# ihsanhadi57/Face-Detection-With-YOLOv11-SAHI-and-Real-ESRGAN

Hardware: AMD Instinct MI355X
Metric: end-to-end 4K frames/sec (SAHI+YOLOv11s+ESRGAN×4) (higher is better)
Workload: dtype f32x3(detect)+f16(sr)

## Files before the change

face-detection-with-yolov11-sahi-and-real-esrgan_amd/build.py:

```python
from __future__ import annotations

import os
import shutil
import subprocess
import sys
from concurrent.futures import ThreadPoolExecutor

HERE = os.path.dirname(os.path.abspath(__file__))
CSRC = os.path.join(HERE, "csrc")
OUT = os.path.join(HERE, "libffp.so")
SOURCES = ["common.cpp", "weights.cpp", "engine.cpp", "conv_route.cpp", "conv_mfma.hip", "conv_rows.hip", "conv_rows16.hip", "conv_rows16pc.hip", "conv_trunk.hip", "conv_pw.hip", "conv_k3d.hip", "conv_dwpw.hip", "ops_misc.hip", "det_post.hip", "merge.hip", "eval.hip", "coco_eval.hip", "iqa.hip", "jpeg.hip", "jpeg_huff.hip", "jpeg_dec.cpp", "png.hip", "png_dec.cpp", "png_dec.hip", "overlay.hip",
           "sr_ops.hip", "resize.hip", "yolo11.cpp", "rrdb.cpp", "onnx_graph.cpp", "scrfd_ops.hip", "scrfd.cpp", "rtdetr_ops.hip", "rtdetr.cpp", "sliced.cpp", "api.cpp",
           "api_eval.cpp", "api_codec.cpp", "api_ops.cpp"]
FLAGS = ["-O3", "-std=c++17", "--offload-arch=gfx950", "-fPIC", "-Wall", "-Wno-unused-function", "-Wno-unused-result",
         "-ffp-contract=off"]


def _hipcc() -> str:
    for c in (os.environ.get("HIPCC"), shutil.which("hipcc"), "/opt/rocm/bin/hipcc"):
        if c and os.path.exists(c):
            return c
    raise RuntimeError("hipcc not found (ROCm toolchain required to build libffp.so)")


# ... 72 lines not shown
        base = _obj_base(s_)
        if s_ in srcs:
            obj = os.path.join(bdir, f"{base}.{name}.o")
            cmd = [_hipcc(), *FLAGS, *defs, "-c", os.path.join(CSRC, s_), "-o", obj]
            r = subprocess.run(cmd, capture_output=True, text=True)
            if r.returncode != 0:
                raise RuntimeError(f"hipcc failed on {s_} ({name}):\n{r.stdout}\n{r.stderr}")
            objs.append(obj)
        else:
            objs.append(os.path.join(bdir, base + ".o"))
    out = os.path.join(bdir, f"libffp_{name}.so")
    r = subprocess.run([_hipcc(), "--offload-arch=gfx950", "-shared", "-fPIC", "-o", out, *objs], capture_output=True, text=True)
    if r.returncode != 0:
        raise RuntimeError(f"link failed:\n{r.stdout}\n{r.stderr}")
    if verbose:
        print(f"built {out}")
    return out


ASAN_SOURCES = ["common.cpp", "weights.cpp", "jpeg_dec.cpp", "png_dec.cpp", "onnx_graph.cpp", "asan_host_check.cpp"]
ASAN_OUT = os.path.join(CSRC, "build", "asan_host_check")


def build_asan(verbose: bool = True) -> str:
    clang = os.path.join(os.path.dirname(os.path.realpath(_hipcc())), "..", "lib", "llvm", "bin", "clang++")
    if not os.path.exists(clang):
        clang = "/opt/rocm/lib/llvm/bin/clang++"
    os.makedirs(os.path.dirname(ASAN_OUT), exist_ok=True)
    srcs = [os.path.join(CSRC, s) for s in ASAN_SOURCES]
    if os.path.exists(ASAN_OUT) and os.path.getmtime(ASAN_OUT) > max(max(os.path.getmtime(s) for s in srcs), _newest_header()):
        return ASAN_OUT
    cmd = [clang, "-std=c++17", "-O1", "-g", "-fsanitize=address,undefined", "-fno-sanitize-recover=undefined", "-fno-omit-frame-pointer",
           "-D__HIP_PLATFORM_AMD__", "-I/opt/rocm/include", *srcs, "-o", ASAN_OUT, "-L/opt/rocm/lib", "-lamdhip64", "-Wl,-rpath,/opt/rocm/lib"]
    r = subprocess.run(cmd, capture_output=True, text=True)
    if r.returncode != 0:
        raise RuntimeError(f"sanitizer build failed:\n{r.stdout}\n{r.stderr}")
    if verbose:
        print(f"built {ASAN_OUT}")
    return ASAN_OUT


def _build_host_check(out: str, driver: str, headers: list, verbose: bool, sanitize: tuple = ("-fsanitize=address,undefined", "-fno-sanitize-recover=undefined")) -> str:
    clang = os.path.join(os.path.dirname(os.path.realpath(_hipcc())), "..", "lib", "llvm", "bin", "clang++")
    if not os.path.exists(clang):
        clang = "/opt/rocm/lib/llvm/bin/clang++"
    out = os.path.join(CSRC, "build", out)
    os.makedirs(os.path.dirname(out), exist_ok=True)
    srcs = [os.path.join(CSRC, f) for f in [driver, *headers]]
    if os.path.exists(out) and os.path.getmtime(out) > max(os.path.getmtime(s) for s in srcs):
        return out
    cmd = [clang, "-std=c++17", "-O1", "-g", "-Wall", *sanitize, "-fno-omit-frame-pointer", srcs[0], "-o", out]
    r = subprocess.run(cmd, capture_output=True, text=True)
    if r.returncode != 0:
        raise RuntimeError(f"sanitizer build failed:\n{r.stdout}\n{r.stderr}")
    if verbose:
        print(f"built {out}")
    return out


def build_arena_check(verbose: bool = True) -> str:
    return _build_host_check("arena_host_check", "arena_host_check.cpp", ["arena.hpp"], verbose)


def build_dw_bound_check(verbose: bool = True) -> str:
    return _build_host_check("dw_bound_host_check", "dw_bound_host_check.cpp", ["dw_bound.hpp"], verbose)


def build_plan_cache_check(verbose: bool = True) -> str:
    return _build_host_check("plan_cache_host_check", "plan_cache_host_check.cpp", ["plan_cache.hpp"], verbose)


def build_switches_check(verbose: bool = True) -> str:
    return _build_host_check("switches_host_check", "switches_host_check.cpp", ["switches.hpp"], verbose)


def build_jpeg_batch_plan_check(verbose: bool = True) -> str:
    return _build_host_check("jpeg_batch_plan_host_check", "jpeg_batch_plan_host_check.cpp", ["jpeg_batch_plan.hpp"], verbose)


def build_sr_tiles_check(verbose: bool = True) -> str:
    return _build_host_check("sr_tiles_host_check", "sr_tiles_host_check.cpp", ["sr_tiles.hpp"], verbose)


def build_ws_pool_check(verbose: bool = True) -> tuple:
    args = ("ws_pool_host_check.cpp", ["ws_pool.hpp"], verbose)
    return (_build_host_check("ws_pool_host_check_asan", *args, sanitize=("-pthread", "-fsanitize=address,undefined", "-fno-sanitize-recover=undefined")),
            _build_host_check("ws_pool_host_check_tsan", *args, sanitize=("-pthread", "-fsanitize=thread")))


if __name__ == "__main__":
    if "--asan" in sys.argv:
        build_asan()
    elif "--arena-check" in sys.argv:
        build_arena_check()
    elif "--dw-bound-check" in sys.argv:
        build_dw_bound_check()
    elif "--plan-cache-check" in sys.argv:
        build_plan_cache_check()
    elif "--switches-check" in sys.argv:
        build_switches_check()
    elif "--jpeg-batch-plan-check" in sys.argv:
        build_jpeg_batch_plan_check()
    elif "--sr-tiles-check" in sys.argv:
        build_sr_tiles_check()
    elif "--ws-pool-check" in sys.argv:
        build_ws_pool_check()
    elif "--variant" in sys.argv:
        build_variant(sys.argv[sys.argv.index("--variant") + 1])
    else:
        build(force="--force" in sys.argv)
```

face-detection-with-yolov11-sahi-and-real-esrgan_amd/csrc/conv_route.cpp:

```cpp
#include "conv_route.hpp"

#include <algorithm>

#include "api_util.hpp"
#include "conv_args.hpp"
#include "engine.hpp"
#include "trunk.hpp"

namespace ffp {

namespace {

using F = ConvFamily;
constexpr ConvShapeInfo kShapes[SHAPE_COUNT] = {
    {SHAPE_WIDE, F::GENERIC, "generic", "wide"},         {SHAPE_WIDE_H, F::GENERIC, "generic", "wideH"},
    {SHAPE_NARROW2, F::GENERIC, "generic", "narrow2"},   {SHAPE_NARROW2_H, F::GENERIC, "generic", "narrow2H"},
    {SHAPE_NARROW1, F::GENERIC, "generic", "narrow1"},   {SHAPE_NARROW1_H, F::GENERIC, "generic", "narrow1H"},
    {SHAPE_ROWS, F::ROWS, "rows", "rows"},               {SHAPE_ROWS_3STAGE, F::ROWS, "rows", "rows"},
    {SHAPE_ROWS_2TILE, F::ROWS, "rows", "rows"},         {SHAPE_ROWS16, F::ROWS16, "rows16", "rows16"},
    {SHAPE_PW_1X4, F::PW, "pw", "pw1x4"},                {SHAPE_PW_2X2, F::PW, "pw", "pw2x2"},
    {SHAPE_PW_2X1, F::PW, "pw", "pw2x1"},                {SHAPE_PW_1X4W, F::PW, "pw", "pw1x4w"},
    {SHAPE_PW_2X2W, F::PW, "pw", "pw2x2w"},              {SHAPE_PW_2X1W, F::PW, "pw", "pw2x1w"},
    {SHAPE_PW_1X4S, F::PW, "pw", "pw1x4s"},              {SHAPE_K3D_128, F::K3D, "k3d", "d128"},
    {SHAPE_K3D_64, F::K3D, "k3d", "d64"},                {SHAPE_K3D_32, F::K3D, "k3d", "d32"},
    {SHAPE_K3D_128X256, F::K3D, "k3d", "d128x256"},      {SHAPE_K3D_64X256, F::K3D, "k3d", "d64x256"},
    {SHAPE_PW_2X2S, F::PW, "pw", "pw2x2s"},              {SHAPE_ROWS16_RES, F::ROWS16, "rows16", "rows16"},
    {SHAPE_ROWS16PC, F::ROWS16PC, "rows16pc", "rows16pc"}, {SHAPE_TRUNK, F::TRUNK, "trunk", "trunk"},
};
constexpr ConvShapeInfo kDwPw{SHAPE_DWPW, F::DWPW, "dwpw", "dw3"};
constexpr bool table_in_order() {
  for (int i = 0; i < SHAPE_COUNT; ++i) if (kShapes[i].shape != i) return false;
  return true;
}
static_assert(table_in_order(), "conv shape table: row i holds shape i");
static_assert(SHAPE_COUNT <= 32 && SHAPE_DWPW >= 32, "forceable shapes fit a 32-bit candidate mask; route-only numbers lie above them");

bool family_runs(ConvFamily family, int shape, const ConvOp& op, const ConvArgs& a) {
  switch (family) {
    case F::GENERIC: return true;
    case F::ROWS: return conv_rows_eligible(op, a, shape);
    case F::ROWS16:
    case F::ROWS16PC: return conv_rows16_eligible(op, a, shape);
    case F::PW: return conv_pw_mask(op, a) & shape_bit(shape);
    case F::K3D: return conv_k3d_mask(op, a) & shape_bit(shape);
    case F::TRUNK: return conv_trunk_layer_ok(op);
    case F::DWPW: return conv_dwpw_eligible(op);
    case F::DIRECT: break;
  }
  return false;
}

}

const ConvShapeInfo* conv_shape_info(int shape) {
  if (shape < 0 || shape >= SHAPE_COUNT) return nullptr;
  return &kShapes[shape];
}

const ConvShapeInfo* conv_route_info(int shape) { return shape == SHAPE_DWPW ? &kDwPw : conv_shape_info(shape); }

ConvArgs conv_route_args(const ConvOp& op) { return op.dw || conv_direct_eligible(op) ? ConvArgs{} : make_conv_args(op); }

ConvRoute conv_route(const ConvOp& op, const ConvArgs& a) {
  if (op.dw) {
    FFP_CHECK((op.force_shape < 0 || op.force_shape == SHAPE_DWPW) && conv_dwpw_eligible(op), FFP_ERR_ARG, "conv %s: the depthwise-fused kernel cannot run this op", op.pc->name.c_str());
    return {F::DWPW, SHAPE_DWPW};
  }
  if (conv_direct_eligible(op)) {
    FFP_CHECK(!op.gate, FFP_ERR_ARG, "conv %s: the image-input kernel cannot honour a gate", op.pc->name.c_str());
    return {F::DIRECT, SHAPE_AUTO};
  }
  if (op.force_shape >= 0) {
    const ConvShapeInfo* s = conv_shape_info(op.force_shape);
    FFP_CHECK(s, FFP_ERR_ARG, "conv %s: %d is not a shape number", op.pc->name.c_str(), op.force_shape);
    FFP_CHECK(family_runs(s->family, s->shape, op, a), FFP_ERR_ARG, "conv %s: %s shape %d cannot run this op", op.pc->name.c_str(), s->family_name, s->shape);
    return {s->family, s->shape};
  }
  if (sw().rows16 && conv_rows16_eligible(op, a, SHAPE_ROWS16)) {
    if (sw().rows16_pc && a.dbg == 0) return {F::ROWS16PC, SHAPE_ROWS16PC};
    if (sw().rows16_res && conv_rows16_eligible(op, a, SHAPE_ROWS16_RES)) return {F::ROWS16, SHAPE_ROWS16_RES};
    return {F::ROWS16, SHAPE_ROWS16};
  }
  if (conv_rows_eligible(op, a, SHAPE_ROWS)) return {F::ROWS, SHAPE_ROWS};
  return {F::GENERIC, conv_generic_choose(op, a)};
}

unsigned conv_candidates(const ConvOp& op, const ConvArgs& a) {
  return conv_generic_mask(op, a) | (sw().pw ? conv_pw_mask(op, a) : 0u) | (sw().k3d ? conv_k3d_mask(op, a) : 0u);
}

void launch_conv(const ConvOp& op, hipStream_t st) {
  ConvArgs a = conv_route_args(op);
  const ConvRoute r = conv_route(op, a);
  switch (r.family) {
    case F::DIRECT: launch_conv_direct(op, st); return;
    case F::GENERIC: launch_conv_generic(a, r.shape, op, st); break;
    case F::ROWS: launch_conv_rows(a, r.shape, op.out.lvl, st); break;
    case F::ROWS16: launch_conv_rows16(a, r.shape, *op.pc, op.out.lvl, st); break;
    case F::ROWS16PC: launch_conv_rows16pc(a, *op.pc, op.out.lvl, st); break;
    case F::PW: launch_conv_pw(a, r.shape, st); break;
    case F::K3D: launch_conv_k3d(a, r.shape, op.stride, op.out.lvl, st); break;
    case F::DWPW: launch_conv_dwpw(op, st); break;
    case F::TRUNK: {
      TrunkPlan tp(std::vector<ConvOp>{op});
      tp.launch(st, op.dbg);
      FFP_HIP(hipStreamSynchronize(st));
      return;
    }
  }
  FFP_HIP(hipGetLastError());
}

std::string conv_variant(const ConvOp& op) {
  const PackedConv& pc = *op.pc;
  const ConvRoute r = conv_route(op, conv_route_args(op));
  if (r.family == F::DIRECT) return std::string(pc.dt == F32 ? "f32" : "f16") + "_k3_direct";
  char buf[64];
  snprintf(buf, sizeof(buf), "%s_k%ds%d_%s", pc.dt == F16 ? "f16" : pc.split ? "f32x3" : "f32", pc.k, op.stride, conv_route_info(r.shape)->suffix);
  return buf;
}

int conv_tune(const ConvOp& op, hipStream_t st) {
  const PackedConv& pc = *op.pc;
  const ConvArgs a = conv_route_args(op);
  const ConvRoute r = conv_route(op, a);
  if (op.force_shape >= 0 || r.family != F::GENERIC) return -1;
  const unsigned mask = conv_candidates(op, a);
  if (__builtin_popcount(mask) < 2) return -1;
  const int heur = r.shape;
  ScopedEvent e0, e1;
  auto time_shape = [&](int shape, int iters) {
    ConvOp o = op;
    o.force_shape = shape;
    o.gate = nullptr;
    FFP_HIP(hipEventRecord(e0, st));
    for (int i = 0; i < iters; ++i) launch_conv(o, st);
    FFP_HIP(hipEventRecord(e1, st));
    FFP_HIP(hipEventSynchronize(e1));
    float ms = 0.f;
    FFP_HIP(hipEventElapsedTime(&ms, e0, e1));
    return ms * 1e3f / iters;
  };
  float best_t = 0.f, heur_t = 0.f;
  int best = -1;
  for (int shape = 0; shape < SHAPE_COUNT; ++shape) {
    if (!(mask & shape_bit(shape))) continue;
    const float t1 = time_shape(shape, 2);
    const int iters = std::min(24, std::max(3, (int)(300.f / std::max(t1, 1.f))));
    const float t = time_shape(shape, iters);
    if (shape == heur) heur_t = t;
    if (best < 0 || t < best_t) { best = shape; best_t = t; }
    if (sw().tune_log) {
      ConvOp o = op;
      o.force_shape = shape;
      fprintf(stderr, "[tune] %-28s %4d->%4d k%d s%d px %9lld  shape %2d %-22s %9.1f us%s\n", pc.name.c_str(), pc.cin_real, pc.cout, pc.k, op.stride,
              (long long)op.out.lvl->actual_px(), shape, conv_variant(o).c_str(), t, shape == heur ? "  (heuristic)" : "");
    }
  }
  if (heur_t > 0.f && best_t > 0.97f * heur_t) return heur;
  return best;
}

}
// ... 1 lines not shown
```

face-detection-with-yolov11-sahi-and-real-esrgan_amd/csrc/conv_route.hpp:

```cpp
#pragma once
#include "ops.hpp"

namespace ffp {

struct ConvArgs;

enum ConvShape : int {
  SHAPE_AUTO = -1,
  SHAPE_WIDE = 0, SHAPE_WIDE_H, SHAPE_NARROW2, SHAPE_NARROW2_H, SHAPE_NARROW1, SHAPE_NARROW1_H,
  SHAPE_ROWS = 6, SHAPE_ROWS_3STAGE, SHAPE_ROWS_2TILE,
  SHAPE_ROWS16 = 9,
  SHAPE_PW_1X4 = 10, SHAPE_PW_2X2, SHAPE_PW_2X1, SHAPE_PW_1X4W, SHAPE_PW_2X2W, SHAPE_PW_2X1W,
  SHAPE_PW_1X4S = 16,
  SHAPE_K3D_128 = 17, SHAPE_K3D_64, SHAPE_K3D_32, SHAPE_K3D_128X256, SHAPE_K3D_64X256,
  SHAPE_PW_2X2S = 22,
  SHAPE_ROWS16_RES = 23,
  SHAPE_ROWS16PC = 24,
  SHAPE_TRUNK = 25,
  SHAPE_COUNT,
  SHAPE_DWPW = 64
};
constexpr unsigned shape_bit(int shape) { return 1u << shape; }

enum class ConvFamily { DIRECT, GENERIC, ROWS, ROWS16, ROWS16PC, PW, K3D, TRUNK, DWPW };

struct ConvShapeInfo { int shape; ConvFamily family; const char* family_name; const char* suffix; };
const ConvShapeInfo* conv_shape_info(int shape);
const ConvShapeInfo* conv_route_info(int shape);

struct ConvRoute { ConvFamily family; int shape; };
ConvRoute conv_route(const ConvOp& op, const ConvArgs& a);
ConvArgs conv_route_args(const ConvOp& op);
unsigned conv_candidates(const ConvOp& op, const ConvArgs& a);

}
```

face-detection-with-yolov11-sahi-and-real-esrgan_amd/csrc/conv_rows16.hip:

```cpp
#include <algorithm>
#include <cstdlib>

#include "rows16_parts.hpp"

#ifndef FFP_R16_DBG
#define FFP_R16_DBG 0
#endif

#ifndef FFP_R16_STAMP
#define FFP_R16_STAMP 0
#endif

namespace ffp {

namespace {

struct R16Lds : R16Geo {
  static constexpr int DESC = 2 * STAGE;
  static constexpr int LDS = 2 * STAGE + TCAP * 48;
  static constexpr int NPR = 6;
  static constexpr int RES_W = 2 * IN_BYTES;
  static constexpr int RES_MAXC = 6;
  static constexpr int res_lds(int nc) { return 2 * IN_BYTES + nc * W_BYTES + TCAP * 48; }
};

template <int DBG, bool RES = false>
__global__ void __launch_bounds__(256, (RES ? 1 : 2)) conv_rows16_kernel(const ConvArgs a) {
  using G = R16Lds;
  constexpr int NP = RES ? G::NPR : G::NP;
  constexpr int STG = RES ? G::IN_BYTES : G::STAGE;
  extern __shared__ __attribute__((aligned(16))) unsigned char smem[];

  const int tid = threadIdx.x, lane = tid & 63;
  const int wave = __builtin_amdgcn_readfirstlane(tid >> 6);
  const int pc = lane & 15, g = lane >> 4;

  const R16Deal deal = r16_deal(a, G::TCAP);
  const int J = deal.J;
  if (J == 0) return;
  const int nt0 = deal.first % a.n_nblk;

  const int NC = a.cin >> 5;
  int4* desc = reinterpret_cast<int4*>(smem + (RES ? G::RES_W + NC * G::W_BYTES : G::DESC));
  r16_fill_desc(desc, a, deal, tid);

  auto sgpr = [](int v) { return __builtin_amdgcn_readfirstlane(v); };
  const unsigned char* wb = reinterpret_cast<const unsigned char*>(a.wpk) + (long long)nt0 * NC * G::W_BYTES;
  const auto rs_w = buf_rsrc(wb);
  auto rs_in = rs_w;
  auto rs_wp = rs_w;

  const bool s9_in = wave == 0;
  const int s9_piece = wave == 0 ? 20 : wave == 1 ? 16 : 17;
  unsigned isrc[6];
  unsigned idst[6];
  unsigned wrel[5];
  unsigned hyx[6];
#pragma unroll
  for (int i = 0; i < 6; ++i) {
    const int idx = (i < 5 ? wave + 4 * i : 20) * 64 + lane;
    const int px = idx >> 2, s = idx & 3;
    const int hy = px / 18, hx = px - hy * 18;
    idst[i] = (unsigned)(px * 64 + ((s ^ ((hx >> 1) & 2)) << 4));
    hyx[i] = px < 324 ? (unsigned)((s << 16) | (hy << 8) | hx) : (unsigned)((s << 16) | 0xFFFF);
  }
#pragma unroll
  for (int i = 0; i < 5; ++i) wrel[i] = (unsigned)(((i < 4 ? wave + 4 * i : s9_piece) * 64 + lane) * 16);

  int pf_item = 0, pf_c = 0;
  int cj = 0, cc = 0;
#if FFP_R16_STAMP
  unsigned long long st_t1 = 0, st_sum[4] = {0, 0, 0, 0};
#endif
  auto setup_pf = [&](int j) {
    const int4 t = desc[j * 3], it = desc[j * 3 + 1];
    const int oy0 = sgpr(t.y), ox0 = sgpr(t.z), Hi = sgpr(it.y), Wi = sgpr(it.z);
    const int Hv = Hi << a.up, Wv = Wi << a.up;
    const unsigned char* inb = reinterpret_cast<const unsigned char*>(a.in) + ((long long)sgpr(it.x) * a.in_cs + a.in_coff) * 2;
    rs_in = buf_rsrc(inb);
#pragma unroll
    for (int i = 0; i < 6; ++i) {
      const int hy = (int)(hyx[i] >> 8) & 0xFF, hx = (int)hyx[i] & 0xFF, sl = (int)(hyx[i] >> 16) & 3;
      const int iy = oy0 - 1 + hy, ix = ox0 - 1 + hx;
      const bool ok = (hyx[i] & 0xFFFFu) != 0xFFFFu && (unsigned)iy < (unsigned)Hv && (unsigned)ix < (unsigned)Wv;
      isrc[i] = ok ? (unsigned)(((iy >> a.up) * Wi + (ix >> a.up)) * a.in_cs * 2 + sl * 16) : BUF_OOB;
// ... 135 lines not shown
    const auto rs_r1 = buf_rsrc(r1b), rs_r2 = buf_rsrc(r2b), rs_o = buf_rsrc(ob);
    const int ox = ox0 + pc;
    const int ch0 = nt0 * 32 + 8 * g;
#pragma unroll
    for (int i = 0; i < 4; ++i) {
      const int oy = oy0 + 4 * wave + i;
      const bool ok = oy < Ho && ox < Wo;
      const unsigned rel_px = (unsigned)(oy * Wo + ox);
      uint4 r1v = make_uint4(0u, 0u, 0u, 0u), r2v = r1v;
      if (a.res1) r1v = buf_load16(rs_r1, ok ? (rel_px * a.r1_cs + ch0) * 2 : BUF_OOB);
      if (a.res2) r2v = buf_load16(rs_r2, ok ? (rel_px * a.r2_cs + ch0) * 2 : BUF_OOB);
      const u32x4 ov = r16_finish_px(acc[i][0], acc[i][1], a.act, a.res1 != nullptr, r1v, a.s1, a.res2 != nullptr, r2v, a.s2);
      __builtin_amdgcn_raw_buffer_store_b128(ov, rs_o, ok ? (rel_px * a.out_cs + ch0) * 2 : BUF_OOB, 0, 0);
    }
  };

  const int Q = J * NC;
  auto finish_chunk = [&]() {
    if (++cc == NC) {
      if (!(DBG & 1)) {
        epilogue(cj);
      } else {
#pragma unroll
        for (int i = 0; i < 4; ++i) asm volatile("" :: "v"(acc[i][0]), "v"(acc[i][1]));
      }
      zero_acc();
      cc = 0; ++cj;
    }
  };
  if constexpr (RES) {
    const int n_wp = NC * 18;
    for (int p0 = wave; p0 < n_wp; p0 += 32) {
      uint4 t[8];
#pragma unroll
      for (int k = 0; k < 8; ++k)
        if (p0 + 4 * k < n_wp) t[k] = buf_load16(rs_w, (unsigned)lane * 16u, sgpr((p0 + 4 * k) << 10));
#pragma unroll
      for (int k = 0; k < 8; ++k)
        if (p0 + 4 * k < n_wp) *reinterpret_cast<uint4*>(smem + G::RES_W + ((p0 + 4 * k) << 10) + lane * 16) = t[k];
    }
  }
  setup_pf(0);
  fetch_all(ra);
  fetch_all(rb);
  stash_all(smem, ra);
  fetch_all(ra);
  __syncthreads();
  for (int q = 0; q < Q; q += 2) {
#if FFP_R16_STAMP
#define R16_PHASES(SB, SBN, SET)                                                      \
    {                                                                                 \
      const unsigned long long t0 = __builtin_amdgcn_s_memtime();                     \
      chunk(SB, SBN, SET);                                                            \
      const unsigned long long t2 = __builtin_amdgcn_s_memtime();                     \
      finish_chunk();                                                                 \
      const unsigned long long t3 = __builtin_amdgcn_s_memtime();                     \
      __syncthreads();                                                                \
      const unsigned long long t4 = __builtin_amdgcn_s_memtime();                     \
      st_sum[0] += st_t1 - t0; st_sum[1] += t2 - st_t1; st_sum[2] += t3 - t2; st_sum[3] += t4 - t3; \
    }
    R16_PHASES(smem, smem + STG, rb)
    if (q + 1 >= Q) break;
    R16_PHASES(smem + STG, smem, ra)
#else
    chunk(smem, smem + STG, rb);
    finish_chunk();
    if (!(DBG & 32)) __syncthreads();
    if (q + 1 >= Q) break;
    chunk(smem + STG, smem, ra);
    finish_chunk();
    if (!(DBG & 32)) __syncthreads();
#endif
  }
#if FFP_R16_STAMP
  if (lane == 0 && (blockIdx.x % 37) == 0 && blockIdx.x < 512)
    printf("r16stamp wg %d wave %d chunks %d items %d : first_frag_reads %llu stream %llu (ideal %d) epilogue+setup %llu barrier %llu cycles per chunk\n", (int)blockIdx.x, wave, Q, J,
           st_sum[0] / Q, st_sum[1] / Q, 72 * 16, st_sum[2] / Q, st_sum[3] / Q);
#endif
}

}

namespace {
#if FFP_R16_DBG
constexpr int kR16Masks[] = {0, 1, 2, 12, 16, 32, 13, 29, 61, 19, 31, 63};
#else
constexpr int kR16Masks[] = {0, 1};
#endif
template <int I = 0> void r16_for_mask(int mask, bool res, bool init, const ConvArgs* a, unsigned grid, int lds, hipStream_t st) {
  if constexpr (I < (int)(sizeof(kR16Masks) / sizeof(int))) {
    if (init) {
      FFP_HIP(hipFuncSetAttribute(reinterpret_cast<const void*>(&conv_rows16_kernel<kR16Masks[I], false>), hipFuncAttributeMaxDynamicSharedMemorySize, R16Lds::LDS));
      FFP_HIP(hipFuncSetAttribute(reinterpret_cast<const void*>(&conv_rows16_kernel<kR16Masks[I], true>), hipFuncAttributeMaxDynamicSharedMemorySize, R16Lds::res_lds(R16Lds::RES_MAXC)));
      r16_for_mask<I + 1>(mask, res, init, a, grid, lds, st);
    } else if (mask == kR16Masks[I]) {
      if (res) hipLaunchKernelGGL((conv_rows16_kernel<kR16Masks[I], true>), dim3(grid), dim3(256), lds, st, *a);
      else hipLaunchKernelGGL((conv_rows16_kernel<kR16Masks[I], false>), dim3(grid), dim3(256), lds, st, *a);
    } else {
      r16_for_mask<I + 1>(mask, res, init, a, grid, lds, st);
    }
  } else if (!init) {
    fail(FFP_ERR_ARG, "rows16: phase-skip mask %d is not built (FFP_R16_DBG)", mask);
  }
}
}

void conv_rows16_init() { r16_for_mask<>(0, false, true, nullptr, 0, 0, nullptr); }

bool conv_rows16_eligible(const ConvOp& op, const ConvArgs& a, int shape) {
  const PackedConv& pc = *op.pc;
  if (shape == SHAPE_ROWS16_RES && (a.cin >> 5) > R16Lds::RES_MAXC) return false;
  return epilogue_fits(op, kEpiR16) && pc.w16.p != nullptr && pc.dt == F16 && pc.k == 3 && op.stride == 1 && pc.cin % 32 == 0 && pc.cin >= 64 && pc.cout % 32 == 0 &&
         pc.cout <= 128 && a.fast_out && op.out.cs % 8 == 0 && op.out.coff % 8 == 0;
}

unsigned rows16_grid(int n_tiles, int n_nblk, int min_ws, int tcap, const char* what) {
  const long long items = (long long)n_tiles * n_nblk;
  long long per_xcd = (items + 7) / 8;
  per_xcd = (per_xcd + n_nblk - 1) / n_nblk * n_nblk;
  long long ws = std::max<long long>(min_ws, (per_xcd + tcap - 1) / tcap);
  ws = (ws + n_nblk - 1) / n_nblk * n_nblk;
  FFP_CHECK(8 * ws < (1ll << 31) && (per_xcd + ws - 1) / ws <= tcap, FFP_ERR_STATE, "%s: launch geometry", what);
  return (unsigned)(8 * ws);
}

void launch_conv_rows16(ConvArgs& a, int shape, const PackedConv& pc, Level* out_lvl, hipStream_t st) {
  using G = R16Lds;
  static_assert(G::LDS <= 80 * 1024, "rows16 kernel: two workgroups per CU");
  a.wpk = pc.w16.p;
  int n_tiles = 0;
  a.tiles = out_lvl->tile_table(16, &n_tiles, &a.n_tiles_dev, st, a.gate);
  if (n_tiles == 0) return;
  a.ntiles_host = n_tiles;
  a.n_nblk = a.ntiles32;
  const bool res = shape == SHAPE_ROWS16_RES;
  const int ws_env = sw().rows16_ws;
  const unsigned grid = rows16_grid(n_tiles, a.n_nblk, ws_env > 0 ? ws_env : (res ? 32 : 64), G::TCAP, "rows16");
  r16_for_mask<>(a.dbg, res, false, &a, grid, res ? G::res_lds(a.cin >> 5) : G::LDS, st);
}

}
```

Before: 147.9.

## Add rows16 kernel computing both 32-channel output blocks per tile for cout=64

Adds a dedicated rows16 convolution kernel for 64-output-channel layers. Each workgroup processes both 32-channel output blocks for a tile, alternating blocks per input-channel chunk, so each staged input tile is reused across both blocks instead of being loaded twice by separate workgroups. A new tail-deal scheme hands leftover tiles to a second half of the grid as single-block half items to balance load. The kernel interleaves staging loads with MFMAs using sched_group_barriers. The cost is more complex routing, an extra kernel variant, and a larger grid.

```diff
diff --git a/face-detection-with-yolov11-sahi-and-real-esrgan_amd/build.py b/face-detection-with-yolov11-sahi-and-real-esrgan_amd/build.py
--- a/face-detection-with-yolov11-sahi-and-real-esrgan_amd/build.py
+++ b/face-detection-with-yolov11-sahi-and-real-esrgan_amd/build.py
@@ -178,6 +178,10 @@
     return _build_host_check("sr_tiles_host_check", "sr_tiles_host_check.cpp", ["sr_tiles.hpp"], verbose)
 
 
+def build_rows16_deal_check(verbose: bool = True) -> str:
+    return _build_host_check("rows16_deal_host_check", "rows16_deal_host_check.cpp", ["rows16_deal.hpp"], verbose)
+
+
 def build_ws_pool_check(verbose: bool = True) -> tuple:
     args = ("ws_pool_host_check.cpp", ["ws_pool.hpp"], verbose)
     return (_build_host_check("ws_pool_host_check_asan", *args, sanitize=("-pthread", "-fsanitize=address,undefined", "-fno-sanitize-recover=undefined")),
@@ -199,6 +203,8 @@
         build_jpeg_batch_plan_check()
     elif "--sr-tiles-check" in sys.argv:
         build_sr_tiles_check()
+    elif "--rows16-deal-check" in sys.argv:
+        build_rows16_deal_check()
     elif "--ws-pool-check" in sys.argv:
         build_ws_pool_check()
     elif "--variant" in sys.argv:
diff --git a/face-detection-with-yolov11-sahi-and-real-esrgan_amd/csrc/conv_route.cpp b/face-detection-with-yolov11-sahi-and-real-esrgan_amd/csrc/conv_route.cpp
--- a/face-detection-with-yolov11-sahi-and-real-esrgan_amd/csrc/conv_route.cpp
+++ b/face-detection-with-yolov11-sahi-and-real-esrgan_amd/csrc/conv_route.cpp
@@ -28,6 +28,7 @@
     {SHAPE_ROWS16PC, F::ROWS16PC, "rows16pc", "rows16pc"}, {SHAPE_TRUNK, F::TRUNK, "trunk", "trunk"},
 };
 constexpr ConvShapeInfo kDwPw{SHAPE_DWPW, F::DWPW, "dwpw", "dw3"};
+constexpr ConvShapeInfo kRows16N64{SHAPE_ROWS16_N64, F::ROWS16, "rows16", "rows16"};
 constexpr bool table_in_order() {
   for (int i = 0; i < SHAPE_COUNT; ++i) if (kShapes[i].shape != i) return false;
   return true;
@@ -57,7 +58,7 @@
   return &kShapes[shape];
 }
 
-const ConvShapeInfo* conv_route_info(int shape) { return shape == SHAPE_DWPW ? &kDwPw : conv_shape_info(shape); }
+const ConvShapeInfo* conv_route_info(int shape) { return shape == SHAPE_DWPW ? &kDwPw : shape == SHAPE_ROWS16_N64 ? &kRows16N64 : conv_shape_info(shape); }
 
 ConvArgs conv_route_args(const ConvOp& op) { return op.dw || conv_direct_eligible(op) ? ConvArgs{} : make_conv_args(op); }
 
@@ -79,6 +80,7 @@
   if (sw().rows16 && conv_rows16_eligible(op, a, SHAPE_ROWS16)) {
     if (sw().rows16_pc && a.dbg == 0) return {F::ROWS16PC, SHAPE_ROWS16PC};
     if (sw().rows16_res && conv_rows16_eligible(op, a, SHAPE_ROWS16_RES)) return {F::ROWS16, SHAPE_ROWS16_RES};
+    if (conv_rows16_eligible(op, a, SHAPE_ROWS16_N64)) return {F::ROWS16, SHAPE_ROWS16_N64};
     return {F::ROWS16, SHAPE_ROWS16};
   }
   if (conv_rows_eligible(op, a, SHAPE_ROWS)) return {F::ROWS, SHAPE_ROWS};
diff --git a/face-detection-with-yolov11-sahi-and-real-esrgan_amd/csrc/conv_route.hpp b/face-detection-with-yolov11-sahi-and-real-esrgan_amd/csrc/conv_route.hpp
--- a/face-detection-with-yolov11-sahi-and-real-esrgan_amd/csrc/conv_route.hpp
+++ b/face-detection-with-yolov11-sahi-and-real-esrgan_amd/csrc/conv_route.hpp
@@ -18,7 +18,8 @@
   SHAPE_ROWS16PC = 24,
   SHAPE_TRUNK = 25,
   SHAPE_COUNT,
-  SHAPE_DWPW = 64
+  SHAPE_DWPW = 64,
+  SHAPE_ROWS16_N64 = 65
 };
 constexpr unsigned shape_bit(int shape) { return 1u << shape; }
 
diff --git a/face-detection-with-yolov11-sahi-and-real-esrgan_amd/csrc/conv_rows16.hip b/face-detection-with-yolov11-sahi-and-real-esrgan_amd/csrc/conv_rows16.hip
--- a/face-detection-with-yolov11-sahi-and-real-esrgan_amd/csrc/conv_rows16.hip
+++ b/face-detection-with-yolov11-sahi-and-real-esrgan_amd/csrc/conv_rows16.hip
@@ -1,6 +1,7 @@
 #include <algorithm>
 #include <cstdlib>
 
+#include "rows16_deal.hpp"
 #include "rows16_parts.hpp"
 
 #ifndef FFP_R16_DBG
@@ -302,6 +303,319 @@
 }
 
 namespace {
+
+struct R16N64Lds : R16Geo {
+  static constexpr int WST = 2 * IN_BYTES;
+  static constexpr int DESC = 2 * IN_BYTES + 2 * W_BYTES;
+  static constexpr int TCAP64 = 32;
+  static constexpr int BIAS = DESC + TCAP64 * 48;
+  static constexpr int LDS = BIAS + 256;
+};
+static_assert(R16N64Lds::LDS <= 80 * 1024, "rows16 64-output form: two workgroups per CU");
+
+__device__ __forceinline__ void r16n64_half_item(const ConvArgs& a, unsigned char* smem, int blk) {
+  using G = R16N64Lds;
+  constexpr int j = 0;
+  const int tid = threadIdx.x, lane = tid & 63;
+  const int wave = __builtin_amdgcn_readfirstlane(tid >> 6);
+  const int pc = lane & 15, g = lane >> 4;
+  const int NC = a.cin >> 5;
+  const int4* desc = reinterpret_cast<const int4*>(smem + G::DESC);
+  auto sgpr = [](int v) { return __builtin_amdgcn_readfirstlane(v); };
+  const unsigned char* wb = reinterpret_cast<const unsigned char*>(a.wpk) + (long long)blk * NC * G::W_BYTES;
+  const auto rs_w = buf_rsrc(wb);
+  auto rs_in = rs_w;
+  unsigned isrc[6], idst[6], wrel[5], hyx[6];
+  r16_stage_tables(wave, lane, idst, hyx, wrel);
+  wrel[4] = (unsigned)(((16 + (wave & 1)) * 64 + lane) * 16);
+  r16_setup_pf(a, desc, j, hyx, isrc, rs_in);
+  uint4 rw[5], ri[6];
+  auto fetch_all = [&](int c) __attribute__((always_inline)) {
+    if (c >= NC) return;
+#pragma unroll
+    for (int i = 0; i < 6; ++i) ri[i] = buf_load16(rs_in, isrc[i] != BUF_OOB ? isrc[i] + (unsigned)(c * 64) : BUF_OOB);
+#pragma unroll
+    for (int p = 0; p < 5; ++p) rw[p] = buf_load16(rs_w, wrel[p], c * G::W_BYTES);
+  };
+  auto stash_all = [&](int st) __attribute__((always_inline)) {
+    unsigned char* sbn = smem + st * G::IN_BYTES;
+    unsigned char* swn = smem + G::WST + st * G::W_BYTES;
+#pragma unroll
+    for (int i = 0; i < 6; ++i) *reinterpret_cast<uint4*>(sbn + idst[i]) = ri[i];
+#pragma unroll
+    for (int p = 0; p < 5; ++p) *reinterpret_cast<uint4*>(swn + wrel[p]) = rw[p];
+  };
+  unsigned boff[3];
+  r16_frag_offsets(4 * wave, pc, g, boff);
+  f32x4 acc[4][2];
+  {
+    const float4* bl = reinterpret_cast<const float4*>(smem + G::BIAS + (blk * 32 + 8 * g) * 4);
+    const float4 b0 = bl[0], b1 = bl[1];
+    r16_zero_acc(acc, b0, b1);
+  }
+  fetch_all(0);
+  stash_all(0);
+  fetch_all(1);
+  __syncthreads();
+  for (int c = 0; c < NC; ++c) {
+    const unsigned char* sb = smem + (c & 1) * G::IN_BYTES;
+    const unsigned char* sw = smem + G::WST + (c & 1) * G::W_BYTES + lane * 16;
+    uint4 bq[2][6], aq[3][2];
+    auto ldB = [&](int kx, int q) {
+#pragma unroll
+      for (int r = 0; r < 6; ++r) bq[q][r] = *reinterpret_cast<const uint4*>(sb + boff[kx] + r * 1152);
+    };
+    auto ldA = [&](int s, int q) {
+      const int tap = (s % 3) * 3 + s / 3;
+#pragma unroll
+      for (int m = 0; m < 2; ++m) aq[q][m] = *reinterpret_cast<const uint4*>(sw + ((tap * 2 + m) << 10));
+    };
+    ldB(0, 0);
+    ldA(0, 0);
+    ldA(1, 1);
+    if (c + 1 < NC) stash_all((c + 1) & 1);
+    fetch_all(c + 2);
+#pragma unroll
+    for (int s = 0; s < 9; ++s) {
+      const int kx = s / 3, ky = s - 3 * kx;
+      if (s + 2 < 9) ldA(s + 2, (s + 2) % 3);
+      if (ky == 0 && kx < 2) ldB(kx + 1, (kx + 1) & 1);
+#pragma unroll
+      for (int i = 0; i < 4; ++i)
+#pragma unroll
+        for (int m = 0; m < 2; ++m) {
+          union { uint4 u; f16x8 h; } ua, ub;
+          ua.u = aq[s % 3][m]; ub.u = bq[kx & 1][i + ky];
+          acc[i][m] = __builtin_amdgcn_mfma_f32_16x16x32_f16(ua.h, ub.h, acc[i][m], 0, 0, 0);
+        }
+    }
+    __syncthreads();
+  }
+  const int4 t = desc[j * 3], ot = desc[j * 3 + 2];
+  const int oy0 = sgpr(t.y), ox0 = sgpr(t.z), Ho = sgpr(ot.y), Wo = sgpr(ot.z);
+  const long long out_base = sgpr(ot.x);
+  const unsigned char* r1b = a.res1 ? reinterpret_cast<const unsigned char*>(a.res1) + (out_base * a.r1_cs + a.r1_coff) * 2 : wb;
+  const unsigned char* r2b = a.res2 ? reinterpret_cast<const unsigned char*>(a.res2) + (out_base * a.r2_cs + a.r2_coff) * 2 : wb;
+  unsigned char* ob = reinterpret_cast<unsigned char*>(a.out) + (out_base * a.out_cs + a.out_coff) * 2;
+  const auto rs_r1 = buf_rsrc(r1b), rs_r2 = buf_rsrc(r2b), rs_o = buf_rsrc(ob);
+  const int ox = ox0 + pc;
+  const int ch0 = blk * 32 + 8 * g;
+#pragma unroll
+  for (int i = 0; i < 4; ++i) {
+    const int oy = oy0 + 4 * wave + i;
+    const bool ok = oy < Ho && ox < Wo;
+    const unsigned rel_px = (unsigned)(oy * Wo + ox);
+    uint4 r1v = make_uint4(0u, 0u, 0u, 0u), r2v = r1v;
+    if (a.res1) r1v = buf_load16(rs_r1, ok ? (rel_px * a.r1_cs + ch0) * 2 : BUF_OOB);
+    if (a.res2) r2v = buf_load16(rs_r2, ok ? (rel_px * a.r2_cs + ch0) * 2 : BUF_OOB);
+    const u32x4 ov = r16_finish_px(acc[i][0], acc[i][1], a.act, a.res1 != nullptr, r1v, a.s1, a.res2 != nullptr, r2v, a.s2);
+    __builtin_amdgcn_raw_buffer_store_b128(ov, rs_o, ok ? (rel_px * a.out_cs + ch0) * 2 : BUF_OOB, 0, 0);
+  }
+}
+
+__global__ void __launch_bounds__(256, 2) conv_rows16n64_kernel(const ConvArgs a) {
+  using G = R16N64Lds;
+  extern __shared__ __attribute__((aligned(16))) unsigned char smem[];
+
+  const int tid = threadIdx.x, lane = tid & 63;
+  const int wave = __builtin_amdgcn_readfirstlane(tid >> 6);
+  const int pc = lane & 15, g = lane >> 4;
+
+  const R16N64Deal deal = r16n64_deal(a.n_tiles_dev ? __builtin_amdgcn_readfirstlane(*a.n_tiles_dev) : a.ntiles_host, (int)blockIdx.x, (int)gridDim.x);
+  const int J = min(deal.items(), G::TCAP64);
+  if (J == 0) return;
+
+  const int NC = a.cin >> 5;
+  int4* desc = reinterpret_cast<int4*>(smem + G::DESC);
+  if (tid < 64) reinterpret_cast<float*>(smem + G::BIAS)[tid] = a.bias[tid];
+  if (tid < J) {
+    const int4 t = a.tiles[deal.tile(tid)];
+    desc[tid * 3] = t;
+    desc[tid * 3 + 1] = a.in_tab[t.x];
+    desc[tid * 3 + 2] = a.out_tab[t.x];
+  }
+  __syncthreads();
+  if (deal.half_blk >= 0) {
+    r16n64_half_item(a, smem, deal.half_blk);
+    return;
+  }
+  const int Jm = J;
+
+  auto sgpr = [](int v) { return __builtin_amdgcn_readfirstlane(v); };
+  const unsigned char* wb = reinterpret_cast<const unsigned char*>(a.wpk);
+  const auto rs_w = buf_rsrc(wb);
+  auto rs_in = rs_w;
+
+  unsigned isrc[6], idst[6];
+  {
+    unsigned hyx[6], wrel[5];
+    r16_stage_tables(wave, lane, idst, hyx, wrel);
+  }
+  const unsigned wl = (unsigned)((wave * 64 + lane) * 16);
+  const unsigned wl4 = (unsigned)(((16 + (wave & 1)) * 64 + lane) * 16);
+
+  int pf_item = 0, pf_c = 0;
+  int cj = 0, cc = 0;
+  uint4 rw[5] = {}, ri[6] = {};
+  auto fetch_in = [&](int i, uint4& r) __attribute__((always_inline)) { r = buf_load16(rs_in, isrc[i] != BUF_OOB ? isrc[i] + (unsigned)(pf_c * 64) : BUF_OOB); };
+  auto fetch_w = [&](int p, uint4& r, int soff) __attribute__((always_inline)) { r = buf_load16(rs_w, p < 4 ? wl : wl4, p < 4 ? soff + 4096 * p : soff); };
+  auto stash_w = [&](unsigned char* sw, int p, const uint4& r) __attribute__((always_inline)) { *reinterpret_cast<uint4*>(sw + (p < 4 ? wl + 4096u * p : wl4)) = r; };
+  auto setup_pf = [&](int j) __attribute__((always_inline)) {
+    const int4 t = desc[j * 3], it = desc[j * 3 + 1];
+    const int oy0 = sgpr(t.y), ox0 = sgpr(t.z), Hi = sgpr(it.y), Wi = sgpr(it.z);
+    const int Hv = Hi << a.up, Wv = Wi << a.up;
+    const unsigned char* inb = reinterpret_cast<const unsigned char*>(a.in) + ((long long)sgpr(it.x) * a.in_cs + a.in_coff) * 2;
+    rs_in = buf_rsrc(inb);
+#pragma unroll
+    for (int i = 0; i < 6; ++i) {
+      const int px = (int)(idst[i] >> 6), hy = (px * 3641) >> 16, hx = px - hy * 18;
+      const int sl = (int)((idst[i] >> 4) & 3) ^ ((hx >> 1) & 2);
+      const int iy = oy0 - 1 + hy, ix = ox0 - 1 + hx;
+      const bool ok = px < 324 && (unsigned)iy < (unsigned)Hv && (unsigned)ix < (unsigned)Wv;
+      isrc[i] = ok ? (unsigned)(((iy >> a.up) * Wi + (ix >> a.up)) * a.in_cs * 2 + sl * 16) : BUF_OOB;
+    }
+  };
+  auto advance_pf = [&]() __attribute__((always_inline)) {
+    if (pf_item >= Jm) return;
+    if (++pf_c == NC) {
+      pf_c = 0;
+      if (++pf_item < Jm) setup_pf(pf_item);
+      else rs_in = buf_rsrc(wb, 0);
+    }
+  };
+
+  unsigned boff[3];
+  r16_frag_offsets(4 * wave, pc, g, boff);
+  const unsigned aoff = lane * 16;
+
+  f32x4 acc[2][4][2];
+  auto zero_acc = [&](int b) __attribute__((always_inline)) {
+    const float4* bl = reinterpret_cast<const float4*>(smem + G::BIAS + (b * 32 + 8 * g) * 4);
+    const float4 b0 = bl[0], b1 = bl[1];
+    r16_zero_acc(acc[b], b0, b1);
+  };
+
+  auto epilogue = [&](int j, int b) __attribute__((always_inline)) {
+    const int4 t = desc[j * 3], ot = desc[j * 3 + 2];
+    const int oy0 = sgpr(t.y), ox0 = sgpr(t.z), Ho = sgpr(ot.y), Wo = sgpr(ot.z);
+    const long long out_base = sgpr(ot.x);
+    const unsigned char* r1b = a.res1 ? reinterpret_cast<const unsigned char*>(a.res1) + (out_base * a.r1_cs + a.r1_coff) * 2 : wb;
+    const unsigned char* r2b = a.res2 ? reinterpret_cast<const unsigned char*>(a.res2) + (out_base * a.r2_cs + a.r2_coff) * 2 : wb;
+    unsigned char* ob = reinterpret_cast<unsigned char*>(a.out) + (out_base * a.out_cs + a.out_coff) * 2;
+    const auto rs_r1 = buf_rsrc(r1b), rs_r2 = buf_rsrc(r2b), rs_o = buf_rsrc(ob);
+    const int ox = ox0 + pc;
+    const int ch0 = b * 32 + 8 * g;
+#pragma unroll
+    for (int i = 0; i < 4; ++i) {
+      const int oy = oy0 + 4 * wave + i;
+      const bool ok = oy < Ho && ox < Wo;
+      const unsigned rel_px = (unsigned)(oy * Wo + ox);
+      uint4 r1v = make_uint4(0u, 0u, 0u, 0u), r2v = r1v;
+      if (a.res1) r1v = buf_load16(rs_r1, ok ? (rel_px * a.r1_cs + ch0) * 2 : BUF_OOB);
+      if (a.res2) r2v = buf_load16(rs_r2, ok ? (rel_px * a.r2_cs + ch0) * 2 : BUF_OOB);
+      const u32x4 ov = r16_finish_px(acc[b][i][0], acc[b][i][1], a.act, a.res1 != nullptr, r1v, a.s1, a.res2 != nullptr, r2v, a.s2);
+      __builtin_amdgcn_raw_buffer_store_b128(ov, rs_o, ok ? (rel_px * a.out_cs + ch0) * 2 : BUF_OOB, 0, 0);
+    }
+  };
+
+  auto half_step = [&](auto BLK, const unsigned char* sb, const unsigned char* sw, unsigned char* sbn, unsigned char* swn) __attribute__((always_inline)) {
+    constexpr int B = decltype(BLK)::value;
+    const int wnext = sgpr((B * NC + (cc + 1 == NC ? 0 : cc + 1)) * G::W_BYTES);
+    auto stage_slot = [&](int s) __attribute__((always_inline)) {
+      if (s < 5) {
+        stash_w(swn, s, rw[s]);
+        fetch_w(s, rw[s], wnext);
+      } else if (s < 8) {
+        const int i = 3 * B + s - 5;
+        *reinterpret_cast<uint4*>(sbn + idst[i]) = ri[i];
+        fetch_in(i, ri[i]);
+      }
+    };
+    uint4 bq[2][6] = {}, aq[3][2] = {};
+    auto ldB = [&](int kx, int q) {
+#pragma unroll
+      for (int j = 0; j < 6; ++j) bq[q][j] = *reinterpret_cast<const uint4*>(sb + boff[kx] + j * 1152);
+    };
+    auto ldA = [&](int s, int q) {
+      const int tap = (s % 3) * 3 + s / 3;
+#pragma unroll
+      for (int m = 0; m < 2; ++m) aq[q][m] = *reinterpret_cast<const uint4*>(sw + aoff + ((tap * 2 + m) << 10));
+    };
+    ldB(0, 0);
+    ldA(0, 0);
+    ldA(1, 1);
+    __builtin_amdgcn_sched_barrier(0);
+#pragma unroll
+    for (int s = 0; s < 9; ++s) {
+      const int kx = s / 3, ky = s - 3 * kx;
+      if (s + 2 < 9) ldA(s + 2, (s + 2) % 3);
+      if (ky == 0 && kx < 2) ldB(kx + 1, (kx + 1) & 1);
+      stage_slot(s);
+#pragma unroll
+      for (int i = 0; i < 4; ++i)
+#pragma unroll
+        for (int m = 0; m < 2; ++m) {
+          union { uint4 u; f16x8 h; } ua, ub;
+          ua.u = aq[s % 3][m]; ub.u = bq[kx & 1][i + ky];
+          acc[B][i][m] = __builtin_amdgcn_mfma_f32_16x16x32_f16(ua.h, ub.h, acc[B][i][m], 0, 0, 0);
+        }
+#pragma unroll
+      for (int r = 0; r < 8; ++r) {
+        __builtin_amdgcn_sched_group_barrier(0x008, 1, 0);
+        __builtin_amdgcn_sched_group_barrier(0x7F6, 2, 0);
+      }
+      __builtin_amdgcn_sched_barrier(0);
+    }
+    if (B == 1) advance_pf();
+    if (cc + 1 == NC) {
+      epilogue(cj, B);
+      zero_acc(B);
+    }
+    if (B == 1 && ++cc == NC) { cc = 0; ++cj; }
+  };
+
+  zero_acc(0);
+  zero_acc(1);
+  setup_pf(0);
+#pragma unroll
+  for (int i = 0; i < 6; ++i) fetch_in(i, ri[i]);
+#pragma unroll
+  for (int p = 0; p < 5; ++p) fetch_w(p, rw[p], 0);
+  advance_pf();
+#pragma unroll
+  for (int i = 0; i < 6; ++i) *reinterpret_cast<uint4*>(smem + idst[i]) = ri[i];
+#pragma unroll
+  for (int p = 0; p < 5; ++p) stash_w(smem + G::WST, p, rw[p]);
+#pragma unroll
+  for (int i = 0; i < 6; ++i) fetch_in(i, ri[i]);
+#pragma unroll
+  for (int p = 0; p < 5; ++p) fetch_w(p, rw[p], sgpr(NC * G::W_BYTES));
+  advance_pf();
+  __syncthreads();
+
+  unsigned char* const in0 = smem;
+  unsigned char* const in1 = smem + G::IN_BYTES;
+  unsigned char* const w0 = smem + G::WST;
+  unsigned char* const w1 = smem + G::WST + G::W_BYTES;
+  using B0 = std::integral_constant<int, 0>;
+  using B1 = std::integral_constant<int, 1>;
+  const int K = Jm * NC;
+  for (int k = 0; k < K; k += 2) {
+    half_step(B0{}, in0, w0, in1, w1);
+    __syncthreads();
+    half_step(B1{}, in0, w1, in1, w0);
+    __syncthreads();
+    if (k + 1 >= K) break;
+    half_step(B0{}, in1, w0, in0, w1);
+    __syncthreads();
+    half_step(B1{}, in1, w1, in0, w0);
+    __syncthreads();
+  }
+}
+
+}
+
+namespace {
 #if FFP_R16_DBG
 constexpr int kR16Masks[] = {0, 1, 2, 12, 16, 32, 13, 29, 61, 19, 31, 63};
 #else
@@ -325,22 +639,22 @@
 }
 }
 
-void conv_rows16_init() { r16_for_mask<>(0, false, true, nullptr, 0, 0, nullptr); }
+void conv_rows16_init() {
+  r16_for_mask<>(0, false, true, nullptr, 0, 0, nullptr);
+  FFP_HIP(hipFuncSetAttribute(reinterpret_cast<const void*>(&conv_rows16n64_kernel), hipFuncAttributeMaxDynamicSharedMemorySize, R16N64Lds::LDS));
+}
 
 bool conv_rows16_eligible(const ConvOp& op, const ConvArgs& a, int shape) {
   const PackedConv& pc = *op.pc;
   if (shape == SHAPE_ROWS16_RES && (a.cin >> 5) > R16Lds::RES_MAXC) return false;
+  if (shape == SHAPE_ROWS16_N64 && (pc.cout != 64 || a.dbg != 0)) return false;
   return epilogue_fits(op, kEpiR16) && pc.w16.p != nullptr && pc.dt == F16 && pc.k == 3 && op.stride == 1 && pc.cin % 32 == 0 && pc.cin >= 64 && pc.cout % 32 == 0 &&
          pc.cout <= 128 && a.fast_out && op.out.cs % 8 == 0 && op.out.coff % 8 == 0;
 }
 
 unsigned rows16_grid(int n_tiles, int n_nblk, int min_ws, int tcap, const char* what) {
-  const long long items = (long long)n_tiles * n_nblk;
-  long long per_xcd = (items + 7) / 8;
-  per_xcd = (per_xcd + n_nblk - 1) / n_nblk * n_nblk;
-  long long ws = std::max<long long>(min_ws, (per_xcd + tcap - 1) / tcap);
-  ws = (ws + n_nblk - 1) / n_nblk * n_nblk;
-  FFP_CHECK(8 * ws < (1ll << 31) && (per_xcd + ws - 1) / ws <= tcap, FFP_ERR_STATE, "%s: launch geometry", what);
+  const long long ws = r16_grid_ws(n_tiles, n_nblk, min_ws, tcap);
+  FFP_CHECK(ws > 0, FFP_ERR_STATE, "%s: launch geometry", what);
   return (unsigned)(8 * ws);
 }
 
@@ -352,9 +666,16 @@
   a.tiles = out_lvl->tile_table(16, &n_tiles, &a.n_tiles_dev, st, a.gate);
   if (n_tiles == 0) return;
   a.ntiles_host = n_tiles;
+  const int ws_env = sw().rows16_ws;
+  if (shape == SHAPE_ROWS16_N64) {
+    a.n_nblk = 1;
+    const unsigned grid = rows16_grid(n_tiles, 1, ws_env > 0 ? ws_env : 64, R16N64Lds::TCAP64, "rows16n64");
+    FFP_CHECK(grid < (1u << 30), FFP_ERR_STATE, "rows16n64: launch geometry");
+    hipLaunchKernelGGL(conv_rows16n64_kernel, dim3(2 * grid), dim3(256), R16N64Lds::LDS, st, a);
+    return;
+  }
   a.n_nblk = a.ntiles32;
   const bool res = shape == SHAPE_ROWS16_RES;
-  const int ws_env = sw().rows16_ws;
   const unsigned grid = rows16_grid(n_tiles, a.n_nblk, ws_env > 0 ? ws_env : (res ? 32 : 64), G::TCAP, "rows16");
   r16_for_mask<>(a.dbg, res, false, &a, grid, res ? G::res_lds(a.cin >> 5) : G::LDS, st);
 }
diff --git a/face-detection-with-yolov11-sahi-and-real-esrgan_amd/csrc/rows16_deal.hpp b/face-detection-with-yolov11-sahi-and-real-esrgan_amd/csrc/rows16_deal.hpp
--- /dev/null
+++ b/face-detection-with-yolov11-sahi-and-real-esrgan_amd/csrc/rows16_deal.hpp
@@ -0,0 +1,51 @@
+#pragma once
+
+#if defined(__HIPCC__)
+#define FFP_R16_HD __host__ __device__ inline
+#else
+#define FFP_R16_HD inline
+#endif
+
+namespace ffp {
+
+FFP_R16_HD long long r16_grid_ws(long long n_tiles, int n_nblk, int min_ws, int tcap) {
+  const long long items = n_tiles * n_nblk;
+  long long per_xcd = (items + 7) / 8;
+  per_xcd = (per_xcd + n_nblk - 1) / n_nblk * n_nblk;
+  long long ws = (per_xcd + tcap - 1) / tcap;
+  if (ws < min_ws) ws = min_ws;
+  ws = (ws + n_nblk - 1) / n_nblk * n_nblk;
+  if (ws < 1 || 8 * ws >= (1ll << 31) || (per_xcd + ws - 1) / ws > tcap) return -1;
+  return ws;
+}
+
+struct R16N64Deal {
+  int first, n_full, Ws;
+  int half_tile, half_blk;
+  FFP_R16_HD int items() const { return half_tile >= 0 ? 1 : n_full; }
+  FFP_R16_HD int tile(int j) const { return half_tile >= 0 ? half_tile : first + j * Ws; }
+};
+FFP_R16_HD R16N64Deal r16n64_deal(int n_tiles, int wg, int n_wg) {
+  R16N64Deal d;
+  d.Ws = n_wg >> 4;
+  const bool second = wg >= 8 * d.Ws;
+  if (second) wg -= 8 * d.Ws;
+  const int xcd = wg & 7, slot = wg >> 3;
+  const int per_xcd = (n_tiles + 7) >> 3;
+  const int base = xcd * per_xcd;
+  const int end = n_tiles < base + per_xcd ? n_tiles : base + per_xcd;
+  const int m = end > base ? end - base : 0;
+  const int rounds = m / d.Ws, r = m - rounds * d.Ws;
+  d.first = base + slot;
+  d.n_full = 0;
+  d.half_tile = d.half_blk = -1;
+  if (!second) {
+    d.n_full = rounds + (2 * r > d.Ws && slot < r ? 1 : 0);
+  } else if (2 * r <= d.Ws && slot < 2 * r) {
+    d.half_tile = base + rounds * d.Ws + (slot >> 1);
+    d.half_blk = slot & 1;
+  }
+  return d;
+}
+
+}
diff --git a/face-detection-with-yolov11-sahi-and-real-esrgan_amd/csrc/rows16_deal_host_check.cpp b/face-detection-with-yolov11-sahi-and-real-esrgan_amd/csrc/rows16_deal_host_check.cpp
--- /dev/null
+++ b/face-detection-with-yolov11-sahi-and-real-esrgan_amd/csrc/rows16_deal_host_check.cpp
@@ -0,0 +1,60 @@
+#include <cstdio>
+#include <vector>
+
+#include "rows16_deal.hpp"
+
+using namespace ffp;
+
+static int fails = 0;
+#define CHECK(c, ...) do { if (!(c)) { if (fails < 20) { std::printf("FAIL %s:%d: ", __FILE__, __LINE__); std::printf(__VA_ARGS__); std::printf("\n"); } ++fails; } } while (0)
+
+constexpr int TCAP = 32;
+
+static void walk(int n_tiles, int ws, std::vector<unsigned char>& seen) {
+  seen.assign((size_t)n_tiles * 2, 0);
+  const int n_wg = 16 * ws;
+  for (int wg = 0; wg < n_wg; ++wg) {
+    const R16N64Deal d = r16n64_deal(n_tiles, wg, n_wg);
+    CHECK(d.Ws == ws, "n %d ws %d wg %d: Ws %d", n_tiles, ws, wg, d.Ws);
+    const int J = d.items();
+    CHECK(J >= 0 && J <= TCAP, "n %d ws %d wg %d: %d items", n_tiles, ws, wg, J);
+    if (d.half_tile >= 0) {
+      CHECK(wg >= 8 * ws && J == 1 && (d.half_blk == 0 || d.half_blk == 1), "n %d ws %d wg %d: half item of block %d, %d items", n_tiles, ws, wg, d.half_blk, J);
+      const int per_xcd = (n_tiles + 7) / 8;
+      CHECK(d.half_tile >= 0 && d.half_tile < n_tiles && d.half_tile / (per_xcd ? per_xcd : 1) == (wg & 7), "n %d ws %d wg %d: half tile %d not of XCD %d", n_tiles, ws, wg, d.half_tile, wg & 7);
+      if (d.half_tile >= 0 && d.half_tile < n_tiles) ++seen[(size_t)d.half_tile * 2 + (d.half_blk & 1)];
+      continue;
+    }
+    CHECK(wg < 8 * ws || J == 0, "n %d ws %d wg %d: full items in the second half", n_tiles, ws, wg);
+    for (int j = 0; j < J; ++j) {
+      const int t = d.tile(j);
+      CHECK(t >= 0 && t < n_tiles, "n %d ws %d wg %d item %d: tile %d", n_tiles, ws, wg, j, t);
+      if (t >= 0 && t < n_tiles) { ++seen[(size_t)t * 2]; ++seen[(size_t)t * 2 + 1]; }
+    }
+  }
+  for (int i = 0; i < 2 * n_tiles; ++i) CHECK(seen[i] == 1, "n %d ws %d: tile %d block %d visited %d times", n_tiles, ws, i / 2, i & 1, (int)seen[i]);
+}
+
+int main() {
+  std::vector<unsigned char> seen;
+  long long launches = 0;
+  for (int n = 0; n <= 6000; ++n) {
+    std::vector<int> wss;
+    auto add = [&](long long cap, int min_ws) {
+      const long long ws = r16_grid_ws(cap, 1, min_ws, TCAP);
+      CHECK(ws >= min_ws && (((cap + 7) / 8) + ws - 1) / ws <= TCAP, "cap %lld min_ws %d: ws %lld", cap, min_ws, ws);
+      if (ws > 0) wss.push_back((int)ws);
+    };
+    add(n, 64);
+    for (int cap = n; cap <= n + n / 2; cap += 1 + n / 8) add(cap, 64);
+    if (n % 7 == 0) for (int w = 1; w <= 1024; w += (w < 130 ? 1 : 97)) add(n, w);
+    for (int ws : wss) { walk(n, ws, seen); ++launches; }
+  }
+  CHECK(r16_grid_ws(1ll << 40, 1, 64, TCAP) == -1, "an impossible launch was accepted");
+  CHECK(r16_grid_ws(0, 1, 64, TCAP) == 64 && r16_grid_ws(8 * 64 * TCAP, 1, 64, TCAP) == 64 && r16_grid_ws(8 * 64 * TCAP + 1, 1, 64, TCAP) == 65, "grid edges");
+  CHECK(r16_grid_ws(5, 2, 3, 40) == 4, "a grid of a two-block layer is a multiple of two");
+  std::printf("%lld launches walked\n", launches);
+  if (fails) { std::printf("rows16_deal_host_check: %d FAILURES\n", fails); return 1; }
+  std::printf("rows16_deal_host_check: ok\n");
+  return 0;
+}
```

Result: no change. 148.8 (median of 6 runs) (+0.6%).
